# elasota/ConvectionKernels

Hardware: AMD Instinct MI355X
Metric: bc7_encode_default_plan_throughput (higher is better)
Workload: dtype f32+u16; 1 GPU; EncodeBC7, BC7EncodingPlan() + Options(), 4096x4096 SplitMix64 random RGBA, seed 2, 1048576 blocks resident in HBM (BASELINE configs[1]); blocks=1048576, exchange=none, search=exact branch-and-bound (output bit-identical)

## Files before the change

convectionkernels_amd/csrc/bc7_kernel.hip:

```cpp
#include <hip/hip_runtime.h>
#include <stdint.h>
#include <float.h>
#include <type_traits>
#include <stdlib.h>

#include "cvtt_device.h"

constexpr int kMaxPTRefine = 2;
constexpr float kBoundGrid16 = 2000.0f, kBoundLimit16 = 2040.0f;
constexpr float kBoundGrid8 = 124.0f, kBoundLimit8 = 127.0f;
#ifndef CVTT_GRID8_RGBA
#define CVTT_GRID8_RGBA true
#endif
#ifndef CVTT_GRID8_RGB
#define CVTT_GRID8_RGB true
#endif
#ifndef CVTT_BC7_WAVES
#define CVTT_BC7_WAVES 4
#endif
#ifndef CVTT_BC7_WAVES_SLOW
#define CVTT_BC7_WAVES_SLOW 4
#endif
#ifndef CVTT_EIG_ITERS
#define CVTT_EIG_ITERS 6
// ... 348 lines not shown
            const float wc = (c == 0) ? A.w[0] : (c == 1) ? A.w[1] : (c == 2) ? A.w[2] : A.w[3];
            u32 sq = 0, su = 0;
            int mn = 255, mx = 0;
            float sw = 0.0f;
#pragma unroll
            for (int g = 0; g < 4; g++)
            {
                sq = __builtin_amdgcn_udot4(mine[g], mine[g], sq, false);
                su = __builtin_amdgcn_udot4(mine[g], 0x01010101u, su, false);
#pragma unroll
                for (int k = 0; k < 4; k++)
                {
                    const int a = byteI(mine[g], k);
                    mn = a < mn ? a : mn;
                    mx = a > mx ? a : mx;
                    sw = sw + byteF(mine[g], k) * wc;
                }
            }
            s_raw[(1 + c) * 16 + (lane >> 2)] = sq;
            s_raw[(5 + c) * 16 + (lane >> 2)] = (u32)mn | ((u32)mx << 8);
            s_raw[(9 + c) * 16 + (lane >> 2)] = __builtin_bit_cast(u32, sw);
            s_raw[(13 + c) * 16 + (lane >> 2)] = __builtin_bit_cast(u32, (float)(int)su);
        }
        __syncthreads();
        auto writeRotatedPixels = [&](int rotation) {
            const uint4 q = *reinterpret_cast<const uint4 *>(&s_pix[lane >> 2][4 * c]);
            *reinterpret_cast<uint4 *>(s_P + 4 * c) = make_uint4(rotatePixel(q.x, rotation), rotatePixel(q.y, rotation),
                                                                 rotatePixel(q.z, rotation), rotatePixel(q.w, rotation));
        };
        int curRotation = FAST ? 0 : -1;
#ifdef CVTT_BC7_PROFILE
        float simKey[12], simErr[12];
        int simN = 0;
#endif
        for (int step = 0; step < 12; step++)
        {
            REFRESH_LANE();
            const int slot = step / 3, which = step - slot * 3;
            const int rotation = (slot == 0) ? rotOrder[0] : (slot == 1) ? rotOrder[1] : (slot == 2) ? rotOrder[2] : rotOrder[3];
            const int mode = which < 2 ? 4 : 5;
            const int indexSelector = which < 2 ? which : 0;
            const int cfg = which < 2 ? rotation * 2 + which : 8 + rotation;
            int numTweak = (mode == 4) ? plan->mode4SP[rotation][indexSelector] : plan->mode5SP[rotation];
            if (numTweak <= 0)
                continue;
            if (numTweak > 4)
                numTweak = 4;
            if (prune)
            {
                const float lb = lbRotOf(rotation);
                if (__ballot(valid && !(lb > work.err)) == 0)
                    continue;
            }

            if (rotation != curRotation)
            {
                if (FAST)
                {
                    __syncthreads();
                    writeRotated(rotation);
                    __syncthreads();
                }
                else
                {
                    __syncthreads();
                    writeRotatedPixels(rotation);
                    __syncthreads();
                }
                curRotation = rotation;
            }
            float rw[4], rwSq[4], rrcpW[4];
#pragma unroll
            for (int ch = 0; ch < 4; ch++)
            {
                rw[ch] = A.w[ch];
                rwSq[ch] = A.wSq[ch];
                rrcpW[ch] = A.rcpW[ch];
            }
#pragma unroll
            for (int ch = 0; ch < 3; ch++)
                if (rotation == ch + 1)
                {
                    rw[ch] = A.w[3];
                    rwSq[ch] = A.wSq[3];
                    rrcpW[ch] = A.rcpW[3];
                    rw[3] = A.w[ch];
                    rwSq[3] = A.wSq[ch];
                    rrcpW[3] = A.rcpW[ch];
                }

            PROF_COUNT(0, 16)
            PROF_COUNT(1, __popcll(__ballot(valid && c == 0 && !(lbRotOf(rotation) > work.err))))
            Unfinished u;
            {
                const UnitRec &ur = s_unit[(lane & ~3) | rotation];
#pragma unroll
                for (int ch = 0; ch < 4; ch++)
                {
                    u.base[ch] = ur.base[ch];
                    u.offset[ch] = ur.offset[ch];
                }
            }
            ShapeBest b, bA;
            {
                DualInv inv;
                const int sepCh = (rotation == 0) ? 3 : rotation - 1;
                inv.words = s_raw + (lane >> 2);
#pragma unroll
                for (int ch = 0; ch < 3; ch++)
                {
                    const int orig = (rotation == ch + 1) ? 3 : ch;
                    inv.rowSq[ch] = (1 + orig) * 16;
                    inv.rowVs[ch] = (9 + orig) * 16;
                }
                inv.rowSq[3] = (1 + sepCh) * 16;
                inv.rowVs[3] = (13 + sepCh) * 16;
                inv.minMax = s_raw[(5 + sepCh) * 16 + (lane >> 2)];
                evalDual<FAST>(s_P, inv, mode, indexSelector, u, numTweak, rw, rwSq, rrcpW, A.flags, T, numRefine, lane, b, bA);
            }

            const float combined = b.err + bA.err;
            const int seq = 384 + cfg;
#ifdef CVTT_BC7_PROFILE
            {
                const float lbp = lbRotOf(rotation);
                const bool needed = valid && c == 0 && !(lbp > work.err);
                PROF_COUNT(6, (needed && (bA.err + lbp > work.err)) ? 1 : 0)
                if (needed && simN < 12)
                {
                    simKey[simN] = lbp + bA.err;
                    simErr[simN] = combined;
                    simN++;
                }
            }
#endif
            if (combined < work.err || (combined == work.err && seq < workSeq))
            {
                work.err = combined;
                workSeq = seq;
                const u32 iLo = indexSelector ? bA.idxLo : b.idxLo, iHi = indexSelector ? bA.idxHi : b.idxHi;
                workPay0 = (c == 0) ? (b.ep0 | bA.ep0) : (c == 3) ? iLo : 0u;
                workPay1 = (c == 0) ? (b.ep1 | bA.ep1) : (c == 3) ? iHi : 0u;
                s_parked[lane >> 2][0] = indexSelector ? b.idxLo : bA.idxLo;
                s_parked[lane >> 2][1] = indexSelector ? b.idxHi : bA.idxHi;
            }
        }
#ifdef CVTT_BC7_PROFILE
        {
            float best = FLT_MAX;
            int evald = 0;
            u32 left = (1u << simN) - 1u;
            while (left)
            {
                int pick = -1;
                float pk = FLT_MAX;
                for (int i = 0; i < 12; i++)
                    if (((left >> i) & 1u) && (pick < 0 || simKey[i] < pk))
                    {
                        pick = i;
                        pk = simKey[i];
                    }
                if (pk > best)
                    break;
                evald++;
                best = simErr[pick] < best ? simErr[pick] : best;
                left &= ~(1u << pick);
            }
            PROF_COUNT(7, evald)
        }
#endif
        __syncthreads();
        PROF_MARK(1)
    }

    auto subsetMaskOf = [&](int numSub, int partition, int sub) -> u32 {
        if (numSub == 1)
            return 0xffffu;
        if (numSub == 2)
        {
            const u32 m1 = s_pm2[partition];
            return sub ? m1 : (~m1 & 0xffffu);
        }
        const u32 m = s_pm3[partition];
        const u32 m1 = m & 0xffffu, m2 = m >> 16;
        return sub == 1 ? m1 : sub == 2 ? m2 : (~(m1 | m2) & 0xffffu);
    };
    auto pixFromLds = [&](u32 (&px)[16]) {
#pragma unroll
        for (int i = 0; i < 4; i++)
        {
            const uint4 v = *reinterpret_cast<const uint4 *>(&s_pix[blk][4 * i]);
            px[4 * i + 0] = v.x;
            px[4 * i + 1] = v.y;
            px[4 * i + 2] = v.z;
            px[4 * i + 3] = v.w;
        }
    };
    enum : int { WS_BOUNDS_FOR = 0, WS_BOUND_BITS = 3, WS_SHARP_RAN = 6, WS_SHARP_NOPAY = 9, WS_T2_NOPAY = 12, WS_STRIKES = 15 };
    u32 ws = (4u << WS_BOUND_BITS) | (4u << WS_SHARP_RAN);
#define WS_GET(f) ((int)((ws >> (f)) & 7u))
#define WS_SET(f, v) do { ws = (u32)__builtin_amdgcn_readfirstlane((int)((ws & ~(7u << (f))) | ((u32)(v) << (f)))); } while (0)
    if (c == 0)
        s_static[blk] = 0.0f;
    if (prune)
    {
        u32 acc = 0;
        u32 lpix[16];
        pixFromLds(lpix);
#pragma unroll
        for (int px = 0; px < 16; px++)
        {
            const int d = 255 - byteI(lpix[px], 3);
            acc = (u32)mad24(d, d, (int)acc);
        }
        if (c == 0)
            s_static[blk] = ((A.flags & CVTTMI_FLAG_UNIFORM) ? (float)(int)acc : (float)(int)acc * A.wSq[3]) * 0.9999f;
    }

    for (int stageOrder = 0; stageOrder < 6; stageOrder++)
    {
        REFRESH_LANE();
        const int stageIter = (ballotA == 0 && !HARD) ? ((stageOrder == 1) ? 2 : (stageOrder == 2) ? 3 : (stageOrder == 3) ? 1 : stageOrder) : stageOrder;
        ModeDesc md;
        int numSubsets, numPartitions, stage, boundSet;
        switch (stageIter)
        {
        case 0: stage = 4; md = {6, 4, 4, 7, 0}; numSubsets = 1; numPartitions = 1; boundSet = 3; break;
        case 1: stage = 5; md = {7, 2, 4, 5, 6}; numSubsets = 2; numPartitions = 64; boundSet = 0; break;
        case 2: stage = 1; md = {1, 3, 2, 6, 7}; numSubsets = 2; numPartitions = 64; boundSet = 1; break;
        case 3: stage = 3; md = {3, 2, 4, 7, 0}; numSubsets = 2; numPartitions = 64; boundSet = 1; break;
        case 4: stage = 0; md = {0, 3, 4, 4, 5}; numSubsets = 3; numPartitions = 16; boundSet = 2; break;
        default: stage = 2; md = {2, 2, 1, 5, 5}; numSubsets = 3; numPartitions = 64; boundSet = 2; break;
        }
        if (HARD && stageIter != 1)
            continue;
        if (stageIter == 1 && ballotA == 0)
            boundSet = 1;
        const int mode = md.mode;
        const bool isRGB = mode < 4;
        const bool laneRuns = isRGB ? allowRGBModes : (mode == 7 ? allowMode7 : true);
        if (__ballot(laneRuns) == 0)
            continue;
        u64 enabled;
        switch (stageIter)
        {
        case 0: enabled = plan->mode6Enabled ? 1 : 0; break;
        case 1: enabled = ~0ull; break;
        case 2: enabled = plan->mode1PartitionEnabled; break;
        case 3: enabled = plan->mode3PartitionEnabled; break;
        case 4: enabled = plan->mode0PartitionEnabled & 0xffffull; break;
        default: enabled = plan->mode2PartitionEnabled; break;
        }
        if (HARD)
            enabled = hardMine;
        if (enabled == 0)
            continue;

        u32 freshAlive = 0;
        bool freshBounds = false;
        if (prune)
        {
            if (WS_GET(WS_BOUNDS_FOR) == boundSet + 1 && WS_GET(WS_BOUND_BITS) < md.indexBits)
                WS_SET(WS_BOUNDS_FOR, 0);
            if (WS_GET(WS_BOUNDS_FOR) != boundSet + 1)
            {
                WS_SET(WS_BOUND_BITS, 4);
                WS_SET(WS_SHARP_RAN, 4);
                __syncthreads();
                if (boundSet == 3)
                {
                }
                else
                {
                    const bool use4 = (boundSet == 0);
                    auto boundsOnGrid = [&](auto g8) {
                    constexpr bool G8 = decltype(g8)::value;
                    const float wsum = A.wSqSum3 + (use4 ? A.wSq[3] : 0.0f);
                    const float scale = (G8 ? kBoundGrid8 : kBoundGrid16) / (255.0f * __builtin_amdgcn_sqrtf(wsum));
                    const float invScaleSq = 1.0f / (scale * scale);
                    const float twoDelta = 2.0f * ((use4 ? A.delta4 : A.delta3) + 0.7072f / scale);
                    const float staticErr = use4 ? 0.0f : s_static[blk];
                    const int rcpLane = (int)kRcpDown[lane < 16 ? lane : 16];
                    auto rcpOf = [&](int n) -> float { return __builtin_bit_cast(float, __builtin_amdgcn_ds_bpermute(n << 2, rcpLane)); };
                    Proj2D<G8> P;
                    PROF_MARK(2)
                    {
                        BlockScatter bsL;
                        {
                            int rs[4], rp[10];
#pragma unroll
                            for (int i = 0; i < 10; i++)
                                rp[i] = s_scatter[blk][i];
#pragma unroll
                            for (int i = 0; i < 4; i++)
                                rs[i] = s_scatter[blk][10 + i];
                            scatterFromRaw(rs, rp, A, bsL);
                        }
                        u32 lpix[16];
                        pixFromLds(lpix);
                        makeProjection(lpix, bsL, A, use4, scale, P);
                    }
                    PROF_MARK(7)
                    const bool two = boundSet < 2;
                    auto selOf = [&](int partition, int which) -> uint4 {
                        return *reinterpret_cast<const uint4 *>(T->subsetByteMask[two ? partition : 64 + 2 * partition + which]);
                    };
                    uint4 selA = make_uint4(0, 0, 0, 0), selB = make_uint4(0, 0, 0, 0);
                    if constexpr (G8)
                    {
                        selA = selOf(c, 0);
                        if (!two)
                            selB = selOf(c, 1);
                    }
                    for (int k = 0; k < 16; k++)
                    {
                        const int partition = 4 * k + c;
                        float lb;
                        uint4 selA1 = selA, selB1 = selB;
                        if constexpr (G8)
                        {
                            const int nextPartition = (k < 15 ? partition + 4 : partition);
                            selA1 = selOf(nextPartition, 0);
                            if (!two)
                                selB1 = selOf(nextPartition, 1);
                        }
                        if (boundSet < 2)
                        {
                            Sums2D s1, s0;
                            if constexpr (G8)
                                maskedSumsSel(P, __popc((u32)s_pm2[partition]), selA, s1);
                            else
                                maskedSums(P, s_pm2[partition], s1);
                            s0.n = 16 - s1.n;
                            s0.u = P.tU - s1.u;
                            s0.v = P.tV - s1.v;
                            s0.uu = P.tUU - s1.uu;
                            s0.vv = P.tVV - s1.vv;
                            s0.uv = P.tUV - s1.uv;
                            lb = subsetBound2D<G8>(s0, rcpOf(s0.n), invScaleSq, twoDelta) + subsetBound2D<G8>(s1, rcpOf(s1.n), invScaleSq, twoDelta);
                        }
                        else
                        {
                            Sums2D s1, s2, s0;
                            if constexpr (G8)
                            {
                                maskedSumsSel(P, __popc(s_pm3[partition] & 0xffffu), selA, s1);
                                maskedSumsSel(P, __popc(s_pm3[partition] >> 16), selB, s2);
                            }
                            else
                            {
                            maskedSums(P, s_pm3[partition] & 0xffffu, s1);
                            maskedSums(P, s_pm3[partition] >> 16, s2);
                            }
                            s0.n = 16 - s1.n - s2.n;
                            s0.u = P.tU - s1.u - s2.u;
                            s0.v = P.tV - s1.v - s2.v;
                            s0.uu = P.tUU - s1.uu - s2.uu;
                            s0.vv = P.tVV - s1.vv - s2.vv;
                            s0.uv = P.tUV - s1.uv - s2.uv;
                            lb = subsetBound2D<G8>(s0, rcpOf(s0.n), invScaleSq, twoDelta) + subsetBound2D<G8>(s1, rcpOf(s1.n), invScaleSq, twoDelta) +
                                 subsetBound2D<G8>(s2, rcpOf(s2.n), invScaleSq, twoDelta);
                        }
                        lb += staticErr;
                        lbStore(partition, blk, lb);
                        freshAlive |= (lb > work.err) ? 0u : (1u << k);
                        selA = selA1;
                        selB = selB1;
                    }
                    freshBounds = true;
                    };
                    if (use4 ? CVTT_GRID8_RGBA : CVTT_GRID8_RGB)
                        boundsOnGrid(std::true_type{});
                    else
                        boundsOnGrid(std::false_type{});
                }
                __syncthreads();
                WS_SET(WS_BOUNDS_FOR, boundSet + 1);
            }
        }
        PROF_MARK(2)

        const int CP = md.numP * 4;
        const int UPB = 64 / CP;
        u32 aliveBits = (valid && laneRuns) ? everyFourth(enabled, c) : 0u;
        if (mode == 7 && anyBlockHasAlpha && !blockHasNonMaxAlpha)
            aliveBits &= everyFourth(mode7RGB, c);
        u32 tier2Done = 0;
        if (prune)
        {
            if (freshBounds)
                aliveBits &= freshAlive;
            else
            {
                for (int k = 0; k * 4 < numPartitions; k++)
                {
                    const float raw = lbLoadRaw(4 * k + c, blk);
                    if (__builtin_fabsf(raw) > work.err)
                        aliveBits &= ~(1u << k);
                    tier2Done |= (__builtin_bit_cast(u32, raw) >> 31) << k;
                }
            }
        }

        if (prune && numSubsets >= 2)
        {
            const bool sharpPays = WS_GET(WS_SHARP_NOPAY) == 0 || md.indexBits < WS_GET(WS_SHARP_NOPAY);
            const u32 todo = aliveBits & ~tier2Done;
            const bool tier2Pays = WS_GET(WS_T2_NOPAY) == 0 || md.indexBits < WS_GET(WS_T2_NOPAY);
            const bool runPlain = tier2Pays && __ballot(todo != 0) != 0;
            const bool maySharp = sharpPays && WS_GET(WS_SHARP_RAN) > md.indexBits;
            if (runPlain || (maySharp && __ballot(aliveBits != 0) != 0))
            {
                const u32 aliveBefore = aliveBits;
                const bool use4 = (boundSet == 0);
                float lw[4];
#pragma unroll
                for (int ch = 0; ch < 4; ch++)
                    lw[ch] = A.w[ch];
                if (runPlain)
                {
                    u32 CM[4][4];
                    {
                        u32 lpix[16];
                        pixFromLds(lpix);
                        channelMajor(lpix, CM);
                    }
                    auto rest = [&](RawSums &d, const RawSums &a) {
                        d.n = 16 - a.n;
#pragma unroll
                        for (int i = 0; i < 4; i++)
                            d.s[i] = s_scatter[blk][10 + i] - a.s[i];
#pragma unroll
                        for (int i = 0; i < 10; i++)
                            d.p[i] = s_scatter[blk][i] - a.p[i];
                    };
                    u32 rem = todo;
                    while (__ballot(rem != 0) != 0)
                    {
                        if (rem != 0)
                        {
                            const int k = __ffs((int)rem) - 1;
                            rem &= rem - 1u;
                            const int partition = 4 * k + c;
                            float lb;
                            RawSums s0, s1;
                            if (numSubsets == 2)
                            {
                                maskedRawSumsCM(CM, s_pm2[partition], s1);
                                rest(s0, s1);
                                lb = use4 ? subsetBoundFull<4>(s1, lw, A.delta4) : subsetBoundFull<3>(s1, lw, A.delta3);
                                lb += use4 ? subsetBoundFull<4>(s0, lw, A.delta4) : subsetBoundFull<3>(s0, lw, A.delta3);
                            }
                            else
                            {
                                maskedRawSumsCM(CM, s_pm3[partition] & 0xffffu, s1);
                                rest(s0, s1);
                                lb = subsetBoundFull<3>(s1, lw, A.delta3);
                                maskedRawSumsCM(CM, s_pm3[partition] >> 16, s1);
                                rawSumsSub(s0, s1);
                                lb += subsetBoundFull<3>(s1, lw, A.delta3);
                                lb += subsetBoundFull<3>(s0, lw, A.delta3);
                            }
                            if (!use4)
                                lb += s_static[blk];
                            lbStoreTier2(partition, blk, fmaxf(lb, lbLoad(partition, blk)));
                            if (lb > work.err)
                                aliveBits &= ~(1u << k);
                        }
                    }
                }
                u32 rem2 = maySharp ? aliveBits : 0u;
                const bool fourLevels = (md.indexBits == 2);
                const int sharpNeed = (numSubsets * (fourLevels ? CVTT_SHARP_COST4 : CVTT_SHARP_COST8) + md.numP * 4 - 1) / (md.numP * 4);
                int sharpCand = __popc(rem2);
#pragma unroll
                for (int step = 1; step < 64; step <<= 1)
                    sharpCand += xorLane(sharpCand, step);
                if (maySharp && sharpCand >= 2 * sharpNeed)
                {
                    const u32 aliveMid = aliveBits;
                    const float wSq3 = A.wSqSum3, wSq4 = A.wSqSum3 + A.wSq[3];
                    WS_SET(WS_SHARP_RAN, md.indexBits);
                    WS_SET(WS_BOUND_BITS, WS_GET(WS_BOUND_BITS) < md.indexBits ? WS_GET(WS_BOUND_BITS) : md.indexBits);
                    bool firstRound = true;
                    while (__ballot(rem2 != 0) != 0)
                    {
                        const bool did = rem2 != 0;
                        bool killed = false;
                        if (did)
                        {
                            const int k = __ffs((int)rem2) - 1;
                            rem2 &= rem2 - 1u;
                            const int partition = 4 * k + c;
                            float lb = 0.0f;
#pragma unroll 1
                            for (int sub = 0; sub < numSubsets; sub++)
                            {
                                const u32 sm = subsetMaskOf(numSubsets, partition, sub);
                                lb += use4 ? subsetBoundSharp<4>(&s_pix[blk][0], sm, lw, A.delta4, wSq4, fourLevels) : subsetBoundSharp<3>(&s_pix[blk][0], sm, lw, A.delta3, wSq3, fourLevels);
                            }
                            if (!use4)
                                lb += s_static[blk];
                            lbStoreTier2(partition, blk, fmaxf(lb, lbLoad(partition, blk)));
                            if (lb > work.err)
                            {
                                aliveBits &= ~(1u << k);
                                killed = true;
                            }
                        }
                        PROF_STAGE2(stageIter, 0, 1)
                        PROF_STAGE2(stageIter, 1, __popcll(__ballot(did)))
                        PROF_STAGE2(stageIter, 2, __popcll(__ballot(killed)))
                        if (__popcll(__ballot(killed)) < sharpNeed)
                        {
                            if (firstRound)
                                WS_SET(WS_SHARP_NOPAY, md.indexBits);
                            break;
                        }
                        firstRound = false;
                    }
                }
                if (runPlain && __ballot(aliveBits != aliveBefore) == 0)
                    WS_SET(WS_T2_NOPAY, md.indexBits);
            }
        }
        if (__ballot(aliveBits != 0) == 0)
            continue;
        if (!PT && !HARD && mode == 7 && A.hardCap != 0)
        {
            int cnt = __popc(aliveBits);
            cnt += xorLane(cnt, 1);
            cnt += xorLane(cnt, 2);
            int waveCnt = cnt;
#pragma unroll
            for (int step = 4; step < 64; step <<= 1)
                waveCnt += xorLane(waveCnt, step);
            u32 allowed = (vGrid - vBlock) / A.hardDiv;
            allowed = allowed > A.hardMin ? allowed : A.hardMin;
            if ((u32)waveCnt >= allowed && cnt >= 2 && (u32)cnt >= allowed / 8u)
            {
                u32 slot = 0;
                if (c == 0)
                    slot = atomicAdd(A.hardCount, 1u);
                slot = __shfl(slot, lane & ~3);
                if (slot < A.hardCap)
                {
                    u64 m = aliveBits;
                    m = (m | (m << 24)) & 0x000000ff000000ffull;
                    m = (m | (m << 12)) & 0x000f000f000f000full;
                    m = (m | (m << 6)) & 0x0303030303030303ull;
                    m = (m | (m << 3)) & 0x1111111111111111ull;
                    m <<= c;
                    u32 lo = (u32)m, hi = (u32)(m >> 32);
                    lo |= xorLane(lo, 1);
                    hi |= xorLane(hi, 1);
                    lo |= xorLane(lo, 2);
                    hi |= xorLane(hi, 2);
                    aliveBits = 0;
                    if (c == 0)
                    {
                        A.hardRec[slot].aliveLo = lo;
                        A.hardRec[slot].aliveHi = hi;
                        s_blkFlags[blk] |= (slot + 1u) << 8;
                    }
                }
            }
        }
        PROF_COUNT(4, __popc(aliveBits))
        PROF_COUNT(5, (c == 0 && valid) ? 1 : 0)
#ifdef CVTT_BC7_PROFILE
        {
            int cntAlive = __popc(aliveBits);
            for (int st = 1; st < 64; st <<= 1) cntAlive += xorLane(cntAlive, st);
            PROF_STAGE(stageIter, 2, cntAlive)
            PROF_STAGE(stageIter, 6, 1)
        }
#endif
        const int itemCap = (numSubsets == 3) ? 21 : 32;
        const bool ptStage = PT && (mode == 6 || mode == 7);
        const bool staged = !ptStage;
        const bool probing = staged && prune && numSubsets >= 2 && (A.prune & 2u) == 0;
        const int offerCap = probing ? 64 : itemCap;
        auto probeSubOf = [&](int partition) -> int {
            if (numSubsets == 2)
                return __popc((u32)s_pm2[partition]) > 8 ? 1 : 0;
            const u32 m = s_pm3[partition];
            const int n1 = __popc(m & 0xffffu), n2 = __popc(m >> 16), n0 = 16 - n1 - n2;
            return (n2 > n0 && n2 > n1) ? 2 : (n1 > n0) ? 1 : 0;
        };
        u64 pend = 0;
        for (;;)
        {
            REFRESH_LANE();
            int numItems = 0, myCount = 0, maxPasses = 1;
            u64 offerMask = 0;
            if (probing)
            {
                u64 m = aliveBits;
                m = (m | (m << 24)) & 0x000000ff000000ffull;
                m = (m | (m << 12)) & 0x000f000f000f000full;
                m = (m | (m << 6)) & 0x0303030303030303ull;
                m = (m | (m << 3)) & 0x1111111111111111ull;
                m <<= c;
                u32 lo = (u32)m, hi = (u32)(m >> 32);
                lo |= xorLane(lo, 1);
                hi |= xorLane(hi, 1);
                lo |= xorLane(lo, 2);
                hi |= xorLane(hi, 2);
                const int kb = __popc(lo) + __popc(hi);
                int allTotal = 0;
#pragma unroll
                for (int b = 0; b < 16; b++)
                    allTotal += __builtin_amdgcn_readlane(kb, 4 * b);
                allTotal = __builtin_amdgcn_readfirstlane(allTotal);
                if (allTotal <= 64)
                {
                    offerMask = ((u64)hi << 32) | lo;
                    aliveBits = 0;
                    numItems = allTotal;
                    maxPasses = 0;
                }
            }
            const bool laneOffers = probing;
            for (int pass = 0; pass < maxPasses; pass++)
            {
                float pickLb = FLT_MAX;
                int pick = 255;
                for (int k = 0; k * 4 < numPartitions; k++)
                {
                    if ((aliveBits >> k) & 1u)
                    {
                        const float lb = prune ? lbLoad(4 * k + c, blk) : 0.0f;
                        if (lb < pickLb)
                        {
                            pickLb = lb;
                            pick = 4 * k + c;
                        }
                    }
                }
                if (!laneOffers)
                {
#pragma unroll
                    for (int step = 1; step <= 2; step <<= 1)
                    {
                        const float oLb = xorLane(pickLb, step);
                        const int oPick = xorLane(pick, step);
                        const bool take = (oLb < pickLb) || (oLb == pickLb && oPick < pick);
                        pickLb = take ? oLb : pickLb;
                        pick = take ? oPick : pick;
                    }
                }
                bool offer = pick < 64 && !(pickLb > work.err);
                if (!offer)
                    aliveBits = 0;
                if (ptStage)
                {
                    if (!offer)
                    {
                        pickLb = FLT_MAX;
                        pick = 255;
                    }
#pragma unroll
                    for (int step = 4; step <= 16; step <<= 1)
                    {
                        const float oLb = xorLane(pickLb, step);
                        const int oPick = xorLane(pick, step);
                        const bool take = (oLb < pickLb) || (oLb == pickLb && oPick < pick);
                        pickLb = take ? oLb : pickLb;
                        pick = take ? oPick : pick;
                    }
// ... 1080 lines not shown
```

Measured before the change: 709.2 Mblocks/s.

## Transpose grid8 bound loop: one partition per lane across all blocks via LDS

In the grid-8 bound computation, each block's projection and totals are staged in shared memory. Each of the 64 lanes then handles one partition and loops over the 16 blocks, instead of each lane walking 16 partitions for its own block. Subset masks, popcounts and reciprocals become per-lane constants loaded once rather than reloaded every iteration. The per-block error is fetched with readlane and alive bits are gathered with ballot. The cost is an extra LDS round trip, an added __syncthreads, and 16 LDS row reads per lane.

```diff
diff --git a/convectionkernels_amd/csrc/bc7_kernel.hip b/convectionkernels_amd/csrc/bc7_kernel.hip
--- a/convectionkernels_amd/csrc/bc7_kernel.hip
+++ b/convectionkernels_amd/csrc/bc7_kernel.hip
@@ -674,35 +674,91 @@
                     }
                     PROF_MARK(7)
                     const bool two = boundSet < 2;
-                    auto selOf = [&](int partition, int which) -> uint4 {
-                        return *reinterpret_cast<const uint4 *>(T->subsetByteMask[two ? partition : 64 + 2 * partition + which]);
+                    if constexpr (G8)
+                    {
+                    u32 *const s_proj = &s_res[0][0];
+                    if (c == 0)
+                    {
+                        uint4 *row = reinterpret_cast<uint4 *>(s_proj + blk * 16);
+                        row[0] = make_uint4(P.U[0], P.U[1], P.U[2], P.U[3]);
+                        row[1] = make_uint4(P.V[0], P.V[1], P.V[2], P.V[3]);
+                        row[2] = make_uint4((u32)P.tU, (u32)P.tV, (u32)P.tUU, (u32)P.tVV);
+                        *reinterpret_cast<uint2 *>(row + 3) = make_uint2((u32)P.tUV, __builtin_bit_cast(u32, staticErr));
+                    }
+                    __syncthreads();
+                    const int partition = lane;
+                    const uint4 selP = *reinterpret_cast<const uint4 *>(T->subsetByteMask[two ? partition : 64 + 2 * partition]);
+                    uint4 selQ = make_uint4(0, 0, 0, 0);
+                    if (!two)
+                        selQ = *reinterpret_cast<const uint4 *>(T->subsetByteMask[64 + 2 * partition + 1]);
+                    const int n1 = two ? __popc((u32)s_pm2[partition]) : __popc(s_pm3[partition] & 0xffffu);
+                    const int n2 = two ? 0 : __popc(s_pm3[partition] >> 16);
+                    const int n0 = 16 - n1 - n2;
+                    const float rcp0 = rcpOf(n0), rcp1 = rcpOf(n1), rcp2 = rcpOf(n2);
+                    const int errBits = __builtin_bit_cast(int, work.err);
+                    u64 alive = 0;
+                    auto trips = [&](auto twoC) {
+                    constexpr bool TWO = decltype(twoC)::value;
+                    auto trip = [&](int b) -> float {
+                        const uint4 *row = reinterpret_cast<const uint4 *>(s_proj + b * 16);
+                        const uint4 ru = row[0], rv = row[1], rt = row[2];
+                        const uint2 rw = *reinterpret_cast<const uint2 *>(row + 3);
+                        Proj2D<true> B;
+                        B.U[0] = ru.x; B.U[1] = ru.y; B.U[2] = ru.z; B.U[3] = ru.w;
+                        B.V[0] = rv.x; B.V[1] = rv.y; B.V[2] = rv.z; B.V[3] = rv.w;
+                        B.tU = (int)rt.x; B.tV = (int)rt.y; B.tUU = (int)rt.z; B.tVV = (int)rt.w; B.tUV = (int)rw.x;
+                        float lb;
+                        Sums2D s1, s0;
+                        maskedSumsSel(B, n1, selP, s1);
+                        if constexpr (TWO)
+                        {
+                            s0.n = n0;
+                            s0.u = B.tU - s1.u;
+                            s0.v = B.tV - s1.v;
+                            s0.uu = B.tUU - s1.uu;
+                            s0.vv = B.tVV - s1.vv;
+                            s0.uv = B.tUV - s1.uv;
+                            lb = subsetBound2D<true>(s0, rcp0, invScaleSq, twoDelta) + subsetBound2D<true>(s1, rcp1, invScaleSq, twoDelta);
+                        }
+                        else
+                        {
+                            Sums2D s2;
+                            maskedSumsSel(B, n2, selQ, s2);
+                            s0.n = n0;
+                            s0.u = B.tU - s1.u - s2.u;
+                            s0.v = B.tV - s1.v - s2.v;
+                            s0.uu = B.tUU - s1.uu - s2.uu;
+                            s0.vv = B.tVV - s1.vv - s2.vv;
+                            s0.uv = B.tUV - s1.uv - s2.uv;
+                            lb = subsetBound2D<true>(s0, rcp0, invScaleSq, twoDelta) + subsetBound2D<true>(s1, rcp1, invScaleSq, twoDelta) +
+                                 subsetBound2D<true>(s2, rcp2, invScaleSq, twoDelta);
+                        }
+                        lb += __builtin_bit_cast(float, rw.y);
+                        const float errB = __builtin_bit_cast(float, __builtin_amdgcn_readlane(errBits, 4 * b));
+                        const u64 aliveB = __ballot(!(lb > errB));
+                        alive = (blk == b) ? aliveB : alive;
+                        return lb;
                     };
-                    uint4 selA = make_uint4(0, 0, 0, 0), selB = make_uint4(0, 0, 0, 0);
-                    if constexpr (G8)
-                    {
-                        selA = selOf(c, 0);
-                        if (!two)
-                            selB = selOf(c, 1);
-                    }
+#pragma unroll
+                    for (int b = 0; b < 16; b++)
+                        lbStore(partition, b, trip(b));
+                    };
+                    if (two)
+                        trips(std::true_type{});
+                    else
+                        trips(std::false_type{});
+                    freshAlive = everyFourth(alive, c);
+                    }
+                    else
+                    {
                     for (int k = 0; k < 16; k++)
                     {
                         const int partition = 4 * k + c;
                         float lb;
-                        uint4 selA1 = selA, selB1 = selB;
-                        if constexpr (G8)
-                        {
-                            const int nextPartition = (k < 15 ? partition + 4 : partition);
-                            selA1 = selOf(nextPartition, 0);
-                            if (!two)
-                                selB1 = selOf(nextPartition, 1);
-                        }
-                        if (boundSet < 2)
+                        if (two)
                         {
                             Sums2D s1, s0;
-                            if constexpr (G8)
-                                maskedSumsSel(P, __popc((u32)s_pm2[partition]), selA, s1);
-                            else
-                                maskedSums(P, s_pm2[partition], s1);
+                            maskedSums(P, s_pm2[partition], s1);
                             s0.n = 16 - s1.n;
                             s0.u = P.tU - s1.u;
                             s0.v = P.tV - s1.v;
@@ -714,16 +770,8 @@
                         else
                         {
                             Sums2D s1, s2, s0;
-                            if constexpr (G8)
-                            {
-                                maskedSumsSel(P, __popc(s_pm3[partition] & 0xffffu), selA, s1);
-                                maskedSumsSel(P, __popc(s_pm3[partition] >> 16), selB, s2);
-                            }
-                            else
-                            {
                             maskedSums(P, s_pm3[partition] & 0xffffu, s1);
                             maskedSums(P, s_pm3[partition] >> 16, s2);
-                            }
                             s0.n = 16 - s1.n - s2.n;
                             s0.u = P.tU - s1.u - s2.u;
                             s0.v = P.tV - s1.v - s2.v;
@@ -736,8 +784,7 @@
                         lb += staticErr;
                         lbStore(partition, blk, lb);
                         freshAlive |= (lb > work.err) ? 0u : (1u << k);
-                        selA = selA1;
-                        selB = selB1;
+                    }
                     }
                     freshBounds = true;
                     };
```

Measured after the change: 714.9 Mblocks/s, median of 6. No clear change (+0.8%).
